# orhosko/tiny-ntt

Hardware: AMD Instinct MI355X
Metric: negacyclic poly-mults/sec (n=4096, 60-bit q), bit-exact vs cg_ntt.py (higher is better)
Workload: dtype u64; 1 GPU; n=4096, q=2^60-2^14+1 (60-bit), global batch 65536 = 65536 rows on this GPU, LCG-seeded rows resident in HBM (BASELINE configs[2]); n=4096, q=1152921504606830593, rows_per_gpu=65536, global_batch=65536, variant=fused, kernel=polymul_fused_kernel, lazy_reduction=True, lib_build_id=280bdc49742b142f, parallelism=batch-sharded x1, no data-path collective

## Files before the change

### __graft_entry__.py

```python
import ctypes
import os
import subprocess
import sys

ROOT = os.path.dirname(os.path.abspath(__file__))
REFERENCE = os.environ.get("TINY_NTT_REFERENCE", "/root/reference")


def _make(directory, *targets):
    cmd = ["make", f"-j{min(8, os.cpu_count() or 1)}", "-C", os.path.join(ROOT, directory), *targets]
    r = subprocess.run(cmd, stdout=subprocess.PIPE, stderr=subprocess.STDOUT, text=True)
    if r.returncode != 0:
        sys.stderr.write(r.stdout)
        raise RuntimeError(f"build failed: {' '.join(cmd)}")


def build() -> None:
    _make("tiny_ntt_amd/csrc")
    _make("oracle", "all")
    _make("tests/emu")
    _make("tests/emu_gadget2")
    _make("tests/devprobe")
    if os.path.isdir(os.path.join(REFERENCE, "software_benchmark")):
        _make("oracle", "ref", f"REFERENCE={REFERENCE}")
    sys.path.insert(0, ROOT)
    import tiny_ntt_amd
    from tiny_ntt_amd import engine
    lib = engine.load_library()
    missing = [s for s in engine.EXPORTED_SYMBOLS if not hasattr(lib, s)]
    if missing:
        raise RuntimeError(f"libtinyntt.so lacks symbols: {missing}")


def smoke() -> None:
    sys.path.insert(0, ROOT)
    import numpy as np
    from tiny_ntt_amd import engine

    n, q, psi = 4096, 1152921504606830593, 431606828070683274
    plan = engine.Plan(n, q, psi, device=0)
    rng = np.random.default_rng(7)
    batch = 4
    a = rng.integers(0, q, size=(batch, n), dtype=np.uint64)
    b = rng.integers(0, q, size=(batch, n), dtype=np.uint64)
    a[0, :] = q - 1
    c = plan.poly_mult(a, b)
    c_cg = plan.poly_mult(a, b, variant="cg8")

    so = os.path.join(ROOT, "oracle", "_build", "liboracle.so")
    if not os.path.exists(so):
        _make("oracle", "all")
    orc = ctypes.CDLL(so)
    P = ctypes.POINTER(ctypes.c_uint64)
    orc.tn_oracle_nwc_poly_mult_batch.argtypes = [P, P, P, ctypes.c_size_t, ctypes.c_size_t, ctypes.c_uint64, ctypes.c_uint64]
    ref = np.empty_like(a)
    rc = orc.tn_oracle_nwc_poly_mult_batch(a.ctypes.data_as(P), b.ctypes.data_as(P), ref.ctypes.data_as(P), batch, n, q, psi)
    assert rc == 0
    assert np.array_equal(c, ref), "fused kernel differs from the oracle"
    assert np.array_equal(c_cg, ref), "cg8 kernel differs from the oracle"
    print(f"smoke ok: n={n} q={q} batch={batch} fused(lazy={plan.is_lazy}) and cg8 bit-exact vs oracle")


if __name__ == "__main__":
    build()
    if len(sys.argv) > 1 and sys.argv[1] == "smoke":
        smoke()
```

### tiny_ntt_amd/csrc/fused_core.h

```cpp
#pragma once
#include <type_traits>
#include "modarith.h"

#ifndef TN_ABL_UNIFORM_TW
#define TN_ABL_UNIFORM_TW 0
#endif

namespace tn {

template <int B, int E_, typename F> struct StaticFor {
  TN_HD static void run(F& f) { f(std::integral_constant<int, B>()); StaticFor<B + 1, E_, F>::run(f); }
};
template <int E_, typename F> struct StaticFor<E_, E_, F> { TN_HD static void run(F&) {} };
template <int B, int E_, typename F> TN_HD void static_for(F&& f) { StaticFor<B, E_, F>::run(f); }

#ifndef TN_FUSED_LPT10
#define TN_FUSED_LPT10 3
#endif
#ifndef TN_FUSED_LPT12
#define TN_FUSED_LPT12 3
#endif
constexpr int fused_lpt(int logn) {
  return logn == 8 ? 2 : logn == 9 ? 3 : logn == 10 ? TN_FUSED_LPT10 : logn == 11 ? 3 : logn == 12 ? TN_FUSED_LPT12 : logn == 13 ? 3 : 0;
}

template <typename E> struct Arith {
  E q;
  u64 mu;
  int k;
  u32 fold_c;
  SplitK sk;
  u64 qmul[17];
  typename TwOf<E>::type one;
  typename TwOf<E>::type ninv;
  typename TwOf<E>::type fninv;
  typename TwOf<E>::type fninv_w1;
  typename TwOf<E>::type bninv;
  typename TwOf<E>::type bninv_w1;
};

template <typename E, int LOGN_, int LPT_> struct FusedCfg {
  static constexpr int LOGN = LOGN_, LPT = LPT_;
  static constexpr int N = 1 << LOGN, R = 1 << LPT, THREADS = N >> LPT;
  static constexpr int PHASES = (LOGN + LPT - 1) / LPT;
  static constexpr int pos(int p) { return (LOGN - (p + 1) * LPT) < 0 ? 0 : (LOGN - (p + 1) * LPT); }
  static constexpr int stage_begin(int p) { return p * LPT; }
  static constexpr int stage_end(int p) { return ((p + 1) * LPT) < LOGN ? ((p + 1) * LPT) : LOGN; }
  static constexpr int ex_pad(int e) { return pos(e + 1) > 0 ? (1 << pos(e + 1)) : 1; }
  static constexpr int ex_sh(int e) { return pos(e + 1) > 0 ? pos(e + 1) + LPT : LPT; }
  static constexpr int lay_span(int e, int cnt) { return cnt + ex_pad(e) * (cnt >> ex_sh(e)); }
  static constexpr int WB = (LOGN - LPT > 6) ? (LOGN - LPT - 6) : 0;
  static constexpr int WSH = LOGN - WB;
  static constexpr int tau_bit_to_j(int p, int t) { return t < pos(p) ? t : t + LPT; }
  static constexpr bool ex_wave_local(int e) {
    for (int t = 6; t < LOGN - LPT; ++t)
      if (tau_bit_to_j(e, t) != t + LPT || tau_bit_to_j(e + 1, t) != t + LPT) return false;
    return true;
  }
  static constexpr int region_elems() {
    int m = 1 << WSH;
    for (int e = 0; e + 1 < PHASES; ++e)
      if (ex_wave_local(e) && lay_span(e, 1 << WSH) > m) m = lay_span(e, 1 << WSH);
    return m;
  }
  static constexpr int lds_elems() {
    int m = region_elems() << WB;
    for (int e = 0; e + 1 < PHASES; ++e)
      if (!ex_wave_local(e) && lay_span(e, N) > m) m = lay_span(e, N);
    return m;
  }
  TN_HD static constexpr u32 jidx(int p, u32 tau, u32 r) {
    return ((tau >> pos(p)) << (pos(p) + LPT)) | (r << pos(p)) | (tau & ((1u << pos(p)) - 1u));
  }
  TN_HD static constexpr u32 prep_idx(u32 tau, u32 r) { return (r << (LOGN - LPT)) | tau; }
  TN_HD static constexpr u32 ex_addr(int e, u32 j) {
    if (WB > 0 && ex_wave_local(e))
      return (j >> WSH) * (u32)region_elems() + (j & ((1u << WSH) - 1u)) + (u32)ex_pad(e) * ((j & ((1u << WSH) - 1u)) >> ex_sh(e));
    return j + (u32)ex_pad(e) * (j >> ex_sh(e));
  }
  TN_HD static constexpr u32 ex_base(int e, int p, u32 tau) { return ex_addr(e, jidx(p, tau, 0)); }
  TN_HD static constexpr u32 ex_off(int e, int p, u32 r) { return ex_addr(e, jidx(p, 0, r)); }
  enum { TW_UNIFORM = 0, TW_WAVE = 1, TW_LDS = 2, TW_REGS = 3, TW_VEC = 4 };
  static constexpr int LDS_TW_MAX_STAGE = 9;
  static constexpr int tw_src(int p) {
    return pos(p) >= LOGN - LPT ? TW_UNIFORM
         : (pos(p) >= 6 ? TW_WAVE : (pos(p) > 0 ? (stage_end(p) <= LDS_TW_MAX_STAGE ? TW_LDS : TW_VEC) : TW_REGS));
  }
  static constexpr int lds_tw_lo() {
    for (int p = 0; p < PHASES; ++p) if (tw_src(p) == TW_LDS) return 1 << stage_begin(p);
    return 0;
  }
  static constexpr int lds_tw_hi() {
    int h = 0;
    for (int p = 0; p < PHASES; ++p) if (tw_src(p) == TW_LDS) h = 1 << stage_end(p);
    return h;
  }
  static constexpr int lds_tw_count() { return lds_tw_hi() - lds_tw_lo(); }
  static constexpr int pre_count(int s) { return R >> ((LOGN - 1 - s) - pos(PHASES - 1) + 1); }
  static constexpr int pre_off(int s) {
    int o = 0;
    for (int i = stage_begin(PHASES - 1); i < s; ++i) o += pre_count(i);
    return o;
  }
  static constexpr int NPRE = (tw_src(PHASES - 1) == TW_REGS) ? pre_off(LOGN) : 1;
  TN_HD static u32 nat_addr(u32 k) { return k ^ ((k >> 5) & 15u); }
  TN_HD static u32 thi(int p, u32 tau) {
    if (pos(p) >= LOGN - LPT) return 0u;
    if (pos(p) >= 6) return wave_uniform(tau >> pos(p));
    return tau >> pos(p);
  }
};

template <typename E> struct LazyTraits;
template <> struct LazyTraits<u64> { static constexpr int LIMIT = 16, TMUL = 4, PW = 2; };
template <> struct LazyTraits<u32> { static constexpr int LIMIT = 64, TMUL = 2, PW = 4; };

template <typename E, bool LAZY, bool CIN = false> struct Policy {
  typedef typename TwOf<E>::type Tw;
  static constexpr bool lazy = LAZY;
  static constexpr bool canonical_inputs = CIN && LAZY && sizeof(E) == 8;
  static constexpr bool split = LAZY && sizeof(E) == 8;
  static constexpr int LIMIT = LazyTraits<E>::LIMIT, TMUL = LazyTraits<E>::TMUL, PW = LazyTraits<E>::PW;

  TN_HD static E load(E x, const Arith<E>& ar) {
    if (canonical_inputs) return x;
    if (LAZY) return fold(x, ar.k, ar.fold_c);
    return mul_tw(x, ar.one, ar.q);
  }
  TN_HD static E canon(E x, const Arith<E>& ar) {
    if (LAZY) { x = fold(x, ar.k, ar.fold_c); return csub(x, ar.q); }
    return x;
  }
  template <int K> TN_HD static void ct(E& u, E& v, Tw w, const Arith<E>& ar) {
    if constexpr (split) {
      const u64 x = mul_sp_acc(u, v, w, ar.sk);
      v = ((u << 1) + ar.qmul[K]) - x;
      u = x;
    } else if constexpr (LAZY) {
      const E t = mul_tw_lazy(v, w, ar.q);
      v = u + ((E)K * ar.q - t);
      u = u + t;
    } else {
      E t = mul_tw(v, w, ar.q);
      E s = u + t;
      v = u >= t ? u - t : u + (ar.q - t);
      u = csub(s, ar.q);
    }
  }
  template <int BND> TN_HD static void gs(E& u, E& v, Tw w, const Arith<E>& ar) {
    if constexpr (split) {
      const E d = (u + ar.qmul[BND]) - v;
      u = u + v;
      v = mul_sp(d, w, ar.sk);
    } else if constexpr (LAZY) {
      const E d = u + ((E)BND * ar.q - v);
      u = u + v;
      v = mul_tw_lazy(d, w, ar.q);
    } else {
      E d = u >= v ? u - v : u + (ar.q - v);
      u = csub(u + v, ar.q);
      v = mul_tw(d, w, ar.q);
    }
  }
  template <int BND> TN_HD static void gs_last(E& u, E& v, const Arith<E>& ar) {
    E d;
    if constexpr (split) d = (u + ar.qmul[BND]) - v;
    else d = LAZY ? (E)(u + ((E)BND * ar.q - v)) : (u >= v ? (E)(u - v) : (E)(u + (ar.q - v)));
    E s = u + v;
    u = mul_tw_canon(s, ar.fninv, ar);
    v = mul_tw_canon(d, ar.fninv_w1, ar);
  }
  TN_HD static E mul_tw_canon(E a, Tw w, const Arith<E>& ar) {
    if constexpr (split) return csub(fold(mul_sp(a, w, ar.sk), ar.k, ar.fold_c), ar.q);
    else return mul_tw(a, w, ar.q);
  }
};

template <typename P, int LOGN> struct Sched {
  static constexpr int fwd_in(int s) {
    int b = 2;
    for (int i = 0; i < s; ++i) { if (b + P::TMUL > P::LIMIT) b = 2; b += P::TMUL; }
    return b;
  }
  static constexpr bool fwd_fold(int s) { return P::lazy && fwd_in(s) + P::TMUL > P::LIMIT; }
  static constexpr int fwd_out() {
    int b = 2;
    for (int i = 0; i < LOGN; ++i) { if (b + P::TMUL > P::LIMIT) b = 2; b += P::TMUL; }
    return b;
  }
  static constexpr int inv_in(int g) {
    int b = P::lazy ? P::PW : 1;
    for (int i = 0; i < g; ++i) { if (2 * b > P::LIMIT) b = 2; b = (2 * b > P::TMUL) ? 2 * b : P::TMUL; }
    return b;
  }
  static constexpr bool inv_fold(int g) { return P::lazy && 2 * inv_in(g) > P::LIMIT; }
  static constexpr int inv_bnd(int g) { return inv_fold(g) ? 2 : inv_in(g); }
};

template <typename Cfg, bool CIN = false, bool BC = false> struct SplitSched {
  static constexpr int LOGN = Cfg::LOGN, R = Cfg::R;
  static constexpr int FEND = BC ? LOGN - 1 : LOGN;
  static constexpr long U = 4096, CAP = 16 * U;
  static constexpr long FOLDED = U + 1;
  static constexpr long PW_OUT = 2 * U;
  static constexpr long PW_IN = 14 * (U - 1);
  static constexpr long tmax(long bv) { return 4 * U + (bv + 7) / 8 + 2; }
  static constexpr long BC_AMAX = CAP - 8;
  static constexpr int kq(long b) { return (int)((b + U - 2) / (U - 1)); }
  static constexpr int kf(long t) { return kq(t) <= 6 ? 6 : kq(t); }
  static constexpr int ki(long b) { return (kq(b) + 3) / 4 * 4; }
  static constexpr int phase_of(int s) { return s / Cfg::LPT; }
  static constexpr int bpos_of(int s) { return (LOGN - 1 - s) - Cfg::pos(phase_of(s)); }
  struct Data {
    bool ffold[LOGN][R] = {};
    unsigned char fk[LOGN][R] = {};
    long fout = 0;
    bool pw_fold_b = false;
    bool bcfold[R] = {};
    bool ifold[LOGN][R] = {};
    unsigned char ik[LOGN][R] = {};
  };
  static constexpr Data build() {
    Data d;
    long b[R] = {};
    for (int r = 0; r < R; ++r) b[r] = CIN ? U : (r < R / 2 ? FOLDED : CAP);
    for (int s = 0; s < FEND; ++s) {
      if (s > 0 && phase_of(s) != phase_of(s - 1)) {
        long m = 0;
        for (int r = 0; r < R; ++r) m = b[r] > m ? b[r] : m;
        for (int r = 0; r < R; ++r) b[r] = m;
      }
      const int bit = 1 << bpos_of(s);
      for (int r = 0; r < R; ++r) {
        if (r & bit) continue;
// ... 325 lines not shown
```

### tiny_ntt_amd/csrc/fused_kernels.h

```cpp
#pragma once
#include <hip/hip_runtime.h>
#include <type_traits>
#include "plan.h"
#include "dev_addr.h"

#ifndef TN_ABL_NO_BARRIER
#define TN_ABL_NO_BARRIER 0
#endif
#ifndef TN_ABL_ROWMASK
#define TN_ABL_ROWMASK 0
#endif
#ifndef TN_ABL_NO_GLOBAL
#define TN_ABL_NO_GLOBAL 0
#endif
#ifndef TN_STORE_AT_TOP
#define TN_STORE_AT_TOP 1
#endif
#ifndef TN_NT_STREAM
#define TN_NT_STREAM 1
#endif
#ifndef TN_FUSED_MIN_WAVES
#define TN_FUSED_MIN_WAVES 4
#endif
#ifndef TN_POLYMUL60_WAVES
#define TN_POLYMUL60_WAVES 6
#endif

#ifndef TN_NTTF_PIN_LOGN
#define TN_NTTF_PIN_LOGN 99
#endif
#ifndef TN_VEC_PREFETCH
#define TN_VEC_PREFETCH 1
#endif
#ifndef TN_FUSED_CIN
#define TN_FUSED_CIN 0
#endif
#ifndef TN_SADDR
#define TN_SADDR 1
#endif
#ifndef TN_KARG_ARITH
#define TN_KARG_ARITH 1
#endif
#ifndef TN_RESIDENT_TW
#define TN_RESIDENT_TW 1
#endif
#ifndef TN_SHARE_MID_TW
#define TN_SHARE_MID_TW 1
#endif
#ifndef TN_SHARE_LAST_TW
#define TN_SHARE_LAST_TW 1
#endif
#ifdef TN_MARKS
#define TN_MARK(n) asm volatile("; TNMARK " n)
#else
#define TN_MARK(n)
#endif
namespace tn {

#ifndef TN_SHUFFLE_LAST
#define TN_SHUFFLE_LAST 0
#endif
template <int DIST> __device__ __forceinline__ u32 lane_xor(u32 v) {
  if constexpr (DIST == 1) return (u32)__builtin_amdgcn_update_dpp(0, (int)v, 0xB1, 0xf, 0xf, false);
  else if constexpr (DIST == 2) return (u32)__builtin_amdgcn_update_dpp(0, (int)v, 0x4E, 0xf, 0xf, false);
  else {
    int r = __builtin_amdgcn_update_dpp(0, (int)v, 0x104, 0xf, 0x5, false);
    return (u32)__builtin_amdgcn_update_dpp(r, (int)v, 0x114, 0xf, 0xA, false);
  }
}
template <typename E>
__device__ __forceinline__ void transpose8_lanes(E (&x)[8], u32 lane) {
  static_for<0, 3>([&](auto b_) {
    constexpr int b = decltype(b_)::value, m = 1 << b;
    const bool hi = (lane >> b) & 1u;
    static_for<0, 8>([&](auto r_) {
      constexpr int r0 = decltype(r_)::value;
      if constexpr (!(r0 & m)) {
        constexpr int r1 = r0 | m;
        const E send = hi ? x[r0] : x[r1];
        E recv;
        if constexpr (sizeof(E) == 8) recv = ((u64)lane_xor<m>((u32)(send >> 32)) << 32) | lane_xor<m>((u32)send);
        else recv = lane_xor<m>((u32)send);
        x[r0] = hi ? recv : x[r0];
        x[r1] = hi ? x[r1] : recv;
      }
    });
  });
}

template <typename E, typename Cfg, int EX, int FROM, int TO>
__device__ __forceinline__ void exchange(E (&x)[Cfg::R], u32 tau, E* lds) {
  if constexpr (TN_SHUFFLE_LAST && Cfg::LPT == 3 && EX == Cfg::PHASES - 2 && Cfg::pos(EX + 1) == 0 && Cfg::pos(EX) == Cfg::LPT) {
    transpose8_lanes<E>(x, tau);
  } else if constexpr (Cfg::ex_wave_local(EX)) {
    __builtin_amdgcn_wave_barrier();
    ex_store<E, Cfg, EX, FROM>(x, tau, lds);
    __builtin_amdgcn_wave_barrier();
    ex_load<E, Cfg, EX, TO>(x, tau, lds);
    __builtin_amdgcn_wave_barrier();
  } else {
#if TN_ABL_NO_BARRIER
    __builtin_amdgcn_wave_barrier();
    ex_store<E, Cfg, EX, FROM>(x, tau, lds);
    __builtin_amdgcn_wave_barrier();
    ex_load<E, Cfg, EX, TO>(x, tau, lds);
    __builtin_amdgcn_wave_barrier();
#else
    __syncthreads();
    ex_store<E, Cfg, EX, FROM>(x, tau, lds);
    __syncthreads();
    ex_load<E, Cfg, EX, TO>(x, tau, lds);
    __syncthreads();
#endif
  }
}

template <typename E>
__device__ __forceinline__ const Arith<E>& kernarg_arith(u32 zero) {
  typedef const __attribute__((address_space(4))) char* KP;
  return *(const Arith<E>*)((KP)__builtin_amdgcn_kernarg_segment_ptr() + zero);
}

template <typename E, typename Cfg, typename Pol, int P0, int P1, bool KARG = false, int PRE_END = Cfg::LOGN, bool BC = false>
__device__ __forceinline__ void forward_range(E (&x)[Cfg::R], u32 tau, const TwRefs<E>& tw_in, const Arith<E>& ar_in, E* lds, bool fetch_pre,
                                              u32 tau_g) {
  typename TwOf<E>::type vec[Cfg::R];
  static_for<P0, P1>([&](auto p_) {
    constexpr int p = decltype(p_)::value;
    constexpr bool FULL = Cfg::stage_end(p) - Cfg::stage_begin(p) == Cfg::LPT;
    TN_MARK("fwd_phase");
    TwRefs<E> tw = tw_in;
    if constexpr (KARG) tw.zero = opaque_zero();
    if constexpr (TN_VEC_PREFETCH && Cfg::tw_src(p) == Cfg::TW_VEC && FULL && p > P0) tw.mid = vec;
    const Arith<E>& ar = KARG ? kernarg_arith<E>(tw.zero) : ar_in;
    fwd_phase<E, Cfg, Pol, p, BC>(x, tau, tw, ar);
    TN_MARK("fwd_other");
    if constexpr (p == Cfg::PHASES - 2) {
      if (fetch_pre) {
        sched_fence();
        tw_prefetch_stages<E, Cfg, Cfg::stage_begin(Cfg::PHASES - 1), PRE_END>(tw.pre, tau_g, tw.glob);
        sched_fence();
      }
    }
    if constexpr (p + 1 < P1) {
      constexpr int pn = p + 1 < Cfg::PHASES ? p + 1 : p;
      if constexpr (TN_VEC_PREFETCH && Cfg::tw_src(pn) == Cfg::TW_VEC && Cfg::stage_end(pn) - Cfg::stage_begin(pn) == Cfg::LPT) {
        sched_fence();
        tw_fetch_vec<E, Cfg, pn>(vec, tau_g, tw.glob);
        sched_fence();
      }
    }
    if constexpr (p + 1 < Cfg::PHASES) exchange<E, Cfg, p, p, p + 1>(x, tau, lds);
  });
}
template <typename E, typename Cfg, typename Pol>
__device__ __forceinline__ void forward_all(E (&x)[Cfg::R], u32 tau, const typename TwOf<E>::type* __restrict__ glob,
                                            const typename TwOf<E>::type* lds_tw, const Arith<E>& ar, E* lds, u32 zero = 0) {
  typename TwOf<E>::type pre[Cfg::NPRE];
  const TwRefs<E> tw = {glob, lds_tw, pre, nullptr, zero};
  forward_range<E, Cfg, Pol, 0, Cfg::PHASES>(x, tau, tw, ar, lds, true, tau);
}

template <typename E, typename Cfg, typename Pol, bool KARG = false, bool BC = false, typename F>
__device__ __forceinline__ void inverse_all(E (&x)[Cfg::R], u32 tau, const TwRefs<E>& tw_in, const Arith<E>& ar_in, E* lds,
                                            F&& after_first) {
  typename TwOf<E>::type vec[Cfg::R];
  static_for<0, Cfg::PHASES>([&](auto i_) {
    constexpr int p = Cfg::PHASES - 1 - decltype(i_)::value;
    constexpr bool FULL = Cfg::stage_end(p) - Cfg::stage_begin(p) == Cfg::LPT;
    TN_MARK("inv_phase");
    TwRefs<E> tw = tw_in;
    if constexpr (KARG) tw.zero = opaque_zero();
    if constexpr (TN_VEC_PREFETCH && Cfg::tw_src(p) == Cfg::TW_VEC && FULL && p < Cfg::PHASES - 1) tw.mid = vec;
    const Arith<E>& ar = KARG ? kernarg_arith<E>(tw.zero) : ar_in;
    inv_phase<E, Cfg, Pol, p, BC>(x, tau, tw, ar);
    TN_MARK("inv_other");
    if constexpr (p > 0) {
      constexpr int pn = p > 0 ? p - 1 : 0;
      if constexpr (TN_VEC_PREFETCH && Cfg::tw_src(pn) == Cfg::TW_VEC && Cfg::stage_end(pn) - Cfg::stage_begin(pn) == Cfg::LPT) {
        sched_fence();
        tw_fetch_vec<E, Cfg, pn>(vec, tau, tw.glob);
        sched_fence();
      }
    }
    if constexpr (p == Cfg::PHASES - 1) { sched_fence(); after_first(); sched_fence(); }
    if constexpr (p > 0) exchange<E, Cfg, p - 1, p, p - 1>(x, tau, lds);
  });
}

template <typename E> struct alignas(2 * sizeof(E)) PairOf { E lo, hi; };

template <typename E, typename Cfg>
__device__ __forceinline__ E ld_operand(const E* __restrict__ p, u32 row, u32 tau, int r) {
#if TN_ABL_NO_GLOBAL
  return (E)(tau * 2654435761u + 7 * r + row);
#else
#if TN_ABL_ROWMASK
  row &= TN_ABL_ROWMASK;
#endif
#if TN_NT_STREAM
  const TN_GLOBAL_AS E* rp = uniform_ptr(p + ((size_t)row << Cfg::LOGN) + Cfg::jidx(0, 0, r));
  return __builtin_nontemporal_load(rp + (Cfg::jidx(0, tau, 0) & (u32)(Cfg::N - 1)));
#else
  return p[((size_t)row << Cfg::LOGN) + Cfg::jidx(0, tau, r)];
#endif
#endif
}

template <typename E, typename Cfg>
__device__ __forceinline__ void st_result(E* __restrict__ c, u32 row, u32 tau, const E (&x)[Cfg::R]) {
#if TN_ABL_ROWMASK
  row &= TN_ABL_ROWMASK;
#endif
  const size_t off = (size_t)row << Cfg::LOGN;
#pragma unroll
  for (int r = 0; r < Cfg::R; ++r) {
#if TN_NT_STREAM
    __builtin_nontemporal_store(x[r], uniform_ptr(c + off + Cfg::jidx(0, 0, r)) + (Cfg::jidx(0, tau, 0) & (u32)(Cfg::N - 1)));
#else
    c[off + Cfg::jidx(0, tau, r)] = x[r];
#endif
  }
}

template <typename E, typename Cfg, bool NT>
__device__ __forceinline__ E ld_prepared(const E* __restrict__ p, u32 row, u32 tau, int r) {
  if constexpr (NT && TN_NT_STREAM) {
    const TN_GLOBAL_AS E* rp = uniform_ptr(p + ((size_t)row << Cfg::LOGN) + Cfg::prep_idx(0, r));
    return __builtin_nontemporal_load(rp + Cfg::prep_idx(tau, 0));
  } else {
    return p[((size_t)row << Cfg::LOGN) + Cfg::prep_idx(tau, r)];
  }
}

template <typename E, int LOGN, int LPT, bool LAZY>
constexpr int polymul_waves() {
  return LPT >= 4 ? 2 : (sizeof(E) == 8 && LOGN == 12 && LAZY) ? TN_POLYMUL60_WAVES : TN_FUSED_MIN_WAVES;
}
#ifndef TN_DOT_WAVES
#define TN_DOT_WAVES 4
#endif
template <typename E, int LOGN, int LPT, bool LAZY>
constexpr int dot_waves() {
  return polymul_waves<E, LOGN, LPT, LAZY>() > TN_DOT_WAVES ? TN_DOT_WAVES : polymul_waves<E, LOGN, LPT, LAZY>();
}

__device__ __forceinline__ void take_next_row(u32& left, u32& chunk_id, u32* lds_next, u32 slot, u32 cur, u32* sched, u32 chunk) {
  if (left) { --left; lds_next[slot] = cur + 1; }
  else {
    chunk_id = sched ? gridDim.x + atomicAdd(&sched[0], 1u) : chunk_id + gridDim.x;
    left = chunk - 1;
    lds_next[slot] = chunk_id * chunk;
  }
}

__device__ __forceinline__ void rearm_row_counters(u32* sched, u32 tau) {
  if (sched && tau == 0 && atomicAdd(&sched[1], 1u) == gridDim.x - 1) { sched[0] = 0; sched[1] = 0; }
}

template <typename E, typename Cfg, typename Pol, bool BC>
__device__ __forceinline__ void dot_last_term(E (&acc)[Cfg::R], E (&xa)[Cfg::R], const E (&xb)[Cfg::R], const typename TwOf<E>::type* zeta,
                                              typename TwOf<E>::type (&pre)[Cfg::NPRE], u32 tl, const typename TwOf<E>::type* tab_inv,
                                              const Arith<E>& ar) {
  if constexpr (BC) {
    basecase<Cfg, Pol>(xa, xb, zeta, ar);
    sched_fence();
    tw_prefetch_stages<E, Cfg, Cfg::stage_begin(Cfg::PHASES - 1), Cfg::LOGN - 1>(pre, tl, tab_inv);
  } else {
    tw_prefetch<E, Cfg>(pre, tl, tab_inv);
    pointwise<E, Cfg, Pol>(xa, xb, ar);
  }
  dot_accumulate<E, Cfg, Pol>(acc, xa, ar);
}

template <bool PRODUCT = false, typename F>
inline hipError_t dispatch_fused_shape(const tn_plan* p, F&& f) {
#ifdef TN_ONLY_MAIN
  if constexpr (PRODUCT) { if (p->elem_bytes == 8 && p->lazy && p->logn == 12) return f(FusedShape<u64, 12, true>()); }
  return hipErrorInvalidValue;
#else
  return with_fused_shape(p->elem_bytes, p->lazy, p->logn, hipErrorInvalidValue, f);
#endif
}

template <typename Sh> struct FusedProductLaunch {
  typedef typename Sh::E E;
  typedef typename TwOf<E>::type Tw;
  static constexpr bool HAS_BC = Sh::HAS_BC;
  const PlanView<E> pv;
  const bool use_bc;
  const FusedProductSetup<E> su;
  explicit FusedProductLaunch(const tn_plan* p, bool cyclic = false, bool no_bc = false)
      : pv(make_view<E>(p)), use_bc(fused_use_bc<Sh>(p->bc_ok, no_bc)), su(fused_product_setup(pv.ar, use_bc, cyclic)) {}
  const Tw* fwd() const { return fused_table(pv, su.fwd); }
  const Tw* inv() const { return fused_table(pv, su.inv); }
};

template <typename Sh>
constexpr size_t fused_lds_bytes(int tables, size_t extra_elems = 0) {
  typedef typename Sh::Cfg Cfg;
  return ((size_t)Cfg::lds_elems() + extra_elems) * sizeof(typename Sh::E) + (size_t)tables * Cfg::lds_tw_count() * sizeof(typename TwOf<typename Sh::E>::type) + 16;
}

}
```

### tiny_ntt_amd/csrc/kernels.hip

```cpp
#include "fused_kernels.h"

namespace tn {

#ifdef TN_FUSED_STAMPS
__device__ unsigned long long tn_fused_stamps[4 * 4096];
#endif

template <typename E, int LOGN, int LPT, bool LAZY, bool CIN = false, bool BC = false>
__global__ void __launch_bounds__((1 << (LOGN - LPT)), (polymul_waves<E, LOGN, LPT, LAZY>()))
polymul_fused_kernel(const Arith<E> ar, const typename TwOf<E>::type* __restrict__ tab_fwd,
                     const typename TwOf<E>::type* __restrict__ tab_inv, const E* __restrict__ a, const E* __restrict__ b,
                     E* __restrict__ c, u32 batch, u32* sched, u32 chunk) {
  typedef FusedCfg<E, LOGN, LPT> Cfg;
  typedef Policy<E, LAZY, CIN> Pol;
  extern __shared__ __attribute__((aligned(16))) unsigned char tn_smem[];
  typedef typename TwOf<E>::type Tw;
  const u32 tau = threadIdx.x;
  E* lds = reinterpret_cast<E*>(tn_smem);
  Tw* lds_fwd = reinterpret_cast<Tw*>(lds + Cfg::lds_elems());
  Tw* lds_inv = lds_fwd + Cfg::lds_tw_count();
  u32* lds_next = reinterpret_cast<u32*>(lds_inv + Cfg::lds_tw_count());
  for (u32 i = tau; i < (u32)Cfg::lds_tw_count(); i += Cfg::THREADS) {
    lds_fwd[i] = tab_fwd[Cfg::lds_tw_lo() + i];
    lds_inv[i] = tab_inv[Cfg::lds_tw_lo() + i];
  }
  __syncthreads();
  E xa[Cfg::R], xb[Cfg::R];
#ifdef TN_FUSED_STAMPS
  const unsigned long long st_t0 = __builtin_amdgcn_s_memtime(), st_r0 = __builtin_amdgcn_s_memrealtime();
#endif
  u32 row = blockIdx.x * chunk;
  u32 taken = 1;
  u32 chunk_id = blockIdx.x;
  if (row < batch) {
#pragma unroll
    for (int r = 0; r < Cfg::R; ++r) xb[r] = ld_operand<E, Cfg>(a, row, tau, r);
  }
  constexpr int PRE_END = (TN_RESIDENT_TW && polymul_waves<E, LOGN, LPT, LAZY>() <= 4 && Cfg::stage_end(Cfg::PHASES - 1) - Cfg::stage_begin(Cfg::PHASES - 1) >= 2) ? Cfg::LOGN - 1 : Cfg::LOGN;
  Tw prf[Cfg::NPRE];
  tw_prefetch_stages<E, Cfg, PRE_END, Cfg::LOGN>(prf, tau, tab_fwd);
  u32 prev = row;
  bool have_c = false;
#pragma unroll
  for (int r = 0; r < Cfg::R; ++r) xa[r] = 0;
  while (row < batch) {
    const u32 zero = opaque_zero();
    const u32 tl = opaque_copy(tau);
    const bool in_chunk = taken != chunk;
    taken = in_chunk ? taken + 1 : 1;
    chunk_id = in_chunk ? chunk_id : chunk_id + gridDim.x;
    if (tau == 0) *lds_next = in_chunk ? row + 1 : (sched ? gridDim.x + atomicAdd(&sched[0], 1u) : chunk_id) * chunk;
    TN_MARK("loop_top");
    E xn[Cfg::R];
#pragma unroll
    for (int r = 0; r < Cfg::R; ++r) xn[r] = xb[r];
    load_reduce<E, Cfg, Pol>(xn, ar);
    sched_fence();
#if TN_STORE_AT_TOP
    st_result<E, Cfg>(c, prev, tl, xa);
#endif
#pragma unroll
    for (int r = 0; r < Cfg::R; ++r) xb[r] = ld_operand<E, Cfg>(b, row, tl, r);
    sched_fence();
#pragma unroll
    for (int r = 0; r < Cfg::R; ++r) xa[r] = xn[r];
    constexpr bool KARG = TN_KARG_ARITH != 0;
    constexpr bool SHARE = TN_SHARE_LAST_TW && Cfg::PHASES >= 2;
    constexpr int PM = Cfg::PHASES >= 3 ? Cfg::PHASES - 2 : 0;
    constexpr bool SHARE2 = SHARE && TN_SHARE_MID_TW && Cfg::PHASES >= 3 && Cfg::tw_src(PM) == Cfg::TW_LDS &&
                            Cfg::stage_end(PM) - Cfg::stage_begin(PM) == Cfg::LPT;
    const TwRefs<E> twf = {tab_fwd, lds_fwd, prf, nullptr, zero};
    static_assert(!BC || SHARE2, "base case: built for the shared-twiddle schedule only");
    if constexpr (SHARE2) forward_range<E, Cfg, Pol, 0, PM, KARG, Cfg::LOGN, BC>(xa, tau, twf, ar, lds, false, tl);
    else if constexpr (SHARE) forward_range<E, Cfg, Pol, 0, Cfg::PHASES - 1, KARG>(xa, tau, twf, ar, lds, false, tl);
    else forward_all<E, Cfg, Pol>(xa, tau, tab_fwd, lds_fwd, ar, lds, zero);
    __syncthreads();
    const u32 next = wave_uniform(*lds_next);
    load_reduce<E, Cfg, Pol>(xb, ar);
    if constexpr (SHARE2) {
      forward_range<E, Cfg, Pol, 0, PM, KARG, Cfg::LOGN, BC>(xb, tau, twf, ar, lds, false, tl);
      Tw mid[Cfg::R];
      tw_fetch_mid<E, Cfg, PM>(mid, tau, lds_fwd);
      const TwRefs<E> twm = {tab_fwd, lds_fwd, prf, mid, zero};
      forward_range<E, Cfg, Pol, PM, PM + 1, KARG, Cfg::LOGN, BC>(xa, tau, twm, ar, lds, false, tl);
      forward_range<E, Cfg, Pol, PM, PM + 1, KARG, PRE_END, BC>(xb, tau, twm, ar, lds, true, tl);
      forward_range<E, Cfg, Pol, PM + 1, Cfg::PHASES, KARG, Cfg::LOGN, BC>(xb, tau, twf, ar, lds, false, tl);
      forward_range<E, Cfg, Pol, PM + 1, Cfg::PHASES, KARG, Cfg::LOGN, BC>(xa, tau, twf, ar, lds, false, tl);
    } else if constexpr (SHARE) {
      forward_range<E, Cfg, Pol, 0, Cfg::PHASES - 1, KARG, PRE_END>(xb, tau, twf, ar, lds, true, tl);
      forward_range<E, Cfg, Pol, Cfg::PHASES - 1, Cfg::PHASES, KARG>(xb, tau, twf, ar, lds, false, tl);
      forward_range<E, Cfg, Pol, Cfg::PHASES - 1, Cfg::PHASES, KARG>(xa, tau, twf, ar, lds, false, tl);
    } else {
      forward_all<E, Cfg, Pol>(xb, tau, tab_fwd, lds_fwd, ar, lds, zero);
    }
    Tw pre[Cfg::NPRE];
    if constexpr (BC) {
      TN_MARK("basecase");
      basecase<Cfg, Pol>(xa, xb, prf + Cfg::pre_off(Cfg::LOGN - 1), ar);
      sched_fence();
      tw_prefetch_stages<E, Cfg, Cfg::stage_begin(Cfg::PHASES - 1), Cfg::LOGN - 1>(pre, tl, tab_inv);
    } else {
      tw_prefetch<E, Cfg>(pre, tl, tab_inv);
      TN_MARK("pointwise");
      pointwise<E, Cfg, Pol>(xa, xb, ar);
    }
    TN_MARK("after_pointwise");
    const TwRefs<E> twi = {tab_inv, lds_inv, pre, nullptr, zero};
    inverse_all<E, Cfg, Pol, KARG, BC>(xa, tau, twi, ar, lds, [&]() {
      const u32 nrow = next < batch ? next : row;
#pragma unroll
      for (int r = 0; r < Cfg::R; ++r) xb[r] = ld_operand<E, Cfg>(a, nrow, tl, r);
    });
#if TN_STORE_AT_TOP
    prev = row;
    have_c = true;
#else
    st_result<E, Cfg>(c, row, tau, xa);
#endif
    row = next;
  }
  if (have_c) st_result<E, Cfg>(c, prev, tau, xa);
#ifdef TN_FUSED_STAMPS
  if (tau == 0 && blockIdx.x < 4096) {
    tn_fused_stamps[4 * blockIdx.x + 0] = st_t0; tn_fused_stamps[4 * blockIdx.x + 1] = st_r0;
    tn_fused_stamps[4 * blockIdx.x + 2] = __builtin_amdgcn_s_memtime(); tn_fused_stamps[4 * blockIdx.x + 3] = __builtin_amdgcn_s_memrealtime();
  }
#endif
  rearm_row_counters(sched, tau);
}

template <typename E, int LOGN, int LPT, bool LAZY, int MODE>
__global__ void __launch_bounds__((1 << (LOGN - LPT)), (LPT >= 4 ? 2 : TN_FUSED_MIN_WAVES))
ntt_fused_kernel(const Arith<E> ar, const typename TwOf<E>::type* __restrict__ tab, const E* __restrict__ in, E* __restrict__ out, u32 batch,
                 u32* sched, u32 chunk) {
  typedef FusedCfg<E, LOGN, LPT> Cfg;
  typedef Policy<E, LAZY> Pol;
  typedef typename TwOf<E>::type Tw;
  extern __shared__ __attribute__((aligned(16))) unsigned char tn_smem[];
  E* lds = reinterpret_cast<E*>(tn_smem);
  const u32 tau = threadIdx.x;
  E* nat = lds + Cfg::lds_elems();
  Tw* lds_tab = reinterpret_cast<Tw*>(nat + Cfg::N);
  u32* lds_next = reinterpret_cast<u32*>(lds_tab + Cfg::lds_tw_count());
  for (u32 i = tau; i < (u32)Cfg::lds_tw_count(); i += Cfg::THREADS) lds_tab[i] = tab[Cfg::lds_tw_lo() + i];
  u32 left = chunk - 1, chunk_id = blockIdx.x;
  if (tau == 0) take_next_row(left, chunk_id, lds_next, 1u, blockIdx.x * chunk, sched, chunk);
  __syncthreads();
  u32 next = wave_uniform(lds_next[1]);
  constexpr int LAST = Cfg::PHASES - 1;
  E xn[Cfg::R];
  u32 row = blockIdx.x * chunk;
  if (row < batch) {
#pragma unroll
    for (int r = 0; r < Cfg::R; ++r) xn[r] = ld_operand<E, Cfg>(in, row, tau, r);
  }
  for (u32 it = 0; row < batch; ++it) {
    if (tau == 0) take_next_row(left, chunk_id, lds_next, it & 1u, next, sched, chunk);
    constexpr bool PIN = LOGN >= TN_NTTF_PIN_LOGN;
    const u32 zero = PIN ? opaque_zero() : 0u;
    const u32 tl = PIN ? opaque_copy(tau) : tau;
    constexpr bool KARG = PIN && TN_KARG_ARITH != 0;
    E x[Cfg::R];
#pragma unroll
    for (int r = 0; r < Cfg::R; ++r) x[r] = xn[r];
    sched_fence();
    if (MODE != FNTT_CYCLIC_INV && next < batch) {
#pragma unroll
      for (int r = 0; r < Cfg::R; ++r) xn[r] = ld_operand<E, Cfg>(in, next, tl, r);
    }
    sched_fence();
    if (MODE == FNTT_CYCLIC_INV) {
#pragma unroll
      for (int r = 0; r < Cfg::R; ++r) x[r] = Pol::load(x[r], ar);
#pragma unroll
      for (int r = 0; r < Cfg::R; ++r) nat[Cfg::nat_addr(Cfg::jidx(0, tau, r))] = x[r];
      __syncthreads();
#pragma unroll
      for (int r = 0; r < Cfg::R; ++r) x[r] = nat[Cfg::nat_addr(bitrev(Cfg::jidx(LAST, tau, r), LOGN))];
      Tw pre[Cfg::NPRE];
      tw_prefetch<E, Cfg>(pre, tl, tab);
      const TwRefs<E> tw = {tab, lds_tab, pre, nullptr, zero};
      inverse_all<E, Cfg, Pol, KARG>(x, tau, tw, ar, lds, [&]() {
        if (next < batch) {
#pragma unroll
          for (int r = 0; r < Cfg::R; ++r) xn[r] = ld_operand<E, Cfg>(in, next, tl, r);
        }
      });
      st_result<E, Cfg>(out, row, tl, x);
    } else {
#pragma unroll
      for (int r = 0; r < Cfg::R / 2; ++r) x[r] = Pol::load(x[r], ar);
      if (!LAZY) {
#pragma unroll
        for (int r = Cfg::R / 2; r < Cfg::R; ++r) x[r] = Pol::load(x[r], ar);
      }
      {
        Tw pre[Cfg::NPRE];
        const TwRefs<E> tw = {tab, lds_tab, pre, nullptr, zero};
        forward_range<E, Cfg, Pol, 0, Cfg::PHASES, KARG>(x, tau, tw, ar, lds, true, tl);
      }
#pragma unroll
      for (int r = 0; r < Cfg::R; ++r)
        nat[Cfg::nat_addr(bitrev(Cfg::jidx(LAST, tau, r), LOGN))] = LAZY ? Pol::canon(x[r], ar) : x[r];
      __syncthreads();
#pragma unroll
      for (int r = 0; r < Cfg::R; ++r) x[r] = nat[Cfg::nat_addr(Cfg::jidx(0, tau, r))];
      st_result<E, Cfg>(out, row, tl, x);
    }
    if (Cfg::THREADS <= 64) __syncthreads();
    row = next;
    next = wave_uniform(lds_next[it & 1u]);
  }
  rearm_row_counters(sched, tau);
}

template <typename Sh>
static hipError_t launch_nttf_t(const tn_plan* p, int mode, const void* in, void* out, size_t batch, hipStream_t s) {
  typedef typename Sh::E E;
  typedef typename Sh::Cfg Cfg;
  typedef typename TwOf<E>::type Tw;
  constexpr int LOGN = Sh::LOGN, LPT = Sh::LPT;
  constexpr bool LAZY = Sh::LAZY;
  constexpr size_t lds_bytes = fused_lds_bytes<Sh>(1, Cfg::N);
  const PlanView<E> pv = make_view<E>(p);
  auto kern = ntt_fused_kernel<E, LOGN, LPT, LAZY, FNTT_TWIST_FWD>;
  if (mode == FNTT_CYCLIC_FWD) kern = ntt_fused_kernel<E, LOGN, LPT, LAZY, FNTT_CYCLIC_FWD>;
  else if (mode != FNTT_TWIST_FWD) kern = ntt_fused_kernel<E, LOGN, LPT, LAZY, FNTT_CYCLIC_INV>;
  const FusedNttSetup<E> su = fused_ntt_setup(pv.ar, mode);
  return launch_persistent(p, s, (const void*)kern, Cfg::THREADS, lds_bytes, Cfg::N * sizeof(E), batch, FUSED_ROWS, [&](u32 grid, u32* sched, u32 chunk) {
    const Tw* tab = fused_table(pv, su.tab);
    const E* in_ = (const E*)in; E* out_ = (E*)out; u32 b32 = (u32)batch;
    Arith<E> ar = su.ar;
    void* args[] = {&ar, &tab, &in_, &out_, &b32, &sched, &chunk};
    return hipLaunchKernel((const void*)kern, dim3(grid), dim3(Cfg::THREADS), args, lds_bytes, s);
  });
}

hipError_t launch_ntt_fused(const tn_plan* p, int mode, const void* in, void* out, size_t batch, hipStream_t s) {
  if (batch == 0) return hipSuccess;
  return dispatch_fused_shape(p, [&](auto sh) { return launch_nttf_t<decltype(sh)>(p, mode, in, out, batch, s); });
}

bool fused_supported(u32 logn, int) { return fused_lpt((int)logn) != 0; }

template <typename Sh>
static hipError_t launch_fused_t(const tn_plan* p, const void* a, const void* b, void* c, size_t batch, hipStream_t s, bool cyclic) {
  typedef typename Sh::E E;
  typedef typename Sh::Cfg Cfg;
  constexpr int LOGN = Sh::LOGN, LPT = Sh::LPT;
  constexpr bool LAZY = Sh::LAZY;
  constexpr size_t lds_bytes = fused_lds_bytes<Sh>(2);
  constexpr bool HAS_CIN = TN_FUSED_CIN && sizeof(E) == 8 && LOGN == 12 && LAZY;
  const bool use_cin = HAS_CIN && p->canonical_inputs && !cyclic;
  const FusedProductLaunch<Sh> L(p, cyclic, use_cin);
  auto kern = polymul_fused_kernel<E, LOGN, LPT, LAZY>;
  if constexpr (HAS_CIN) { if (use_cin) kern = polymul_fused_kernel<E, LOGN, LPT, LAZY, true>; }
  if constexpr (L.HAS_BC) { if (L.use_bc) kern = polymul_fused_kernel<E, LOGN, LPT, LAZY, false, true>; }
  return launch_persistent(p, s, reinterpret_cast<const void*>(kern), Cfg::THREADS, lds_bytes, Cfg::N * sizeof(E), batch, FUSED_ROWS,
                           [&](u32 grid, u32* sched, u32 chunk) {
    hipLaunchKernelGGL(kern, dim3(grid), dim3(Cfg::THREADS), lds_bytes, s, L.su.ar, L.fwd(), L.inv(),
                       (const E*)a, (const E*)b, (E*)c, (u32)batch, sched, chunk);
// ... 183 lines not shown
```

Before: 30.12 million poly-mults/s.

## Drop redundant block barriers around cross-wave LDS transposes in polymul row

```diff
diff --git a/__graft_entry__.py b/__graft_entry__.py
--- a/__graft_entry__.py
+++ b/__graft_entry__.py
@@ -20,6 +20,7 @@
     _make("oracle", "all")
     _make("tests/emu")
     _make("tests/emu_gadget2")
+    _make("tests/emu_sync")
     _make("tests/devprobe")
     if os.path.isdir(os.path.join(REFERENCE, "software_benchmark")):
         _make("oracle", "ref", f"REFERENCE={REFERENCE}")
diff --git a/tiny_ntt_amd/csrc/fused_core.h b/tiny_ntt_amd/csrc/fused_core.h
--- a/tiny_ntt_amd/csrc/fused_core.h
+++ b/tiny_ntt_amd/csrc/fused_core.h
@@ -6,6 +6,9 @@
 #define TN_ABL_UNIFORM_TW 0
 #endif
 
+#ifndef TN_PRODUCT_SYNC
+#define TN_PRODUCT_SYNC 1
+#endif
 namespace tn {
 
 template <int B, int E_, typename F> struct StaticFor {
@@ -80,6 +83,53 @@
   }
   TN_HD static constexpr u32 ex_base(int e, int p, u32 tau) { return ex_addr(e, jidx(p, tau, 0)); }
   TN_HD static constexpr u32 ex_off(int e, int p, u32 r) { return ex_addr(e, jidx(p, 0, r)); }
+  enum { EXB_BEFORE = 1, EXB_BETWEEN = 2, EXB_AFTER = 4, EXB_ALL = 7 };
+  static constexpr bool side_region_local_eval(int e, int p) {
+    const bool local = WB > 0 && ex_wave_local(e);
+    const u32 region = (u32)region_elems(), pad = (u32)ex_pad(e), low = (1u << WSH) - 1u;
+    const int sh = ex_sh(e);
+    for (u32 tau = 0; tau < (u32)THREADS; ++tau)
+      for (u32 r = 0; r < (u32)R; ++r) {
+        const u32 j = jidx(p, tau, r), w = tau >> 6;
+        const u32 a = local ? (j >> WSH) * region + (j & low) + pad * ((j & low) >> sh) : j + pad * (j >> sh);
+        if (a < w * region || a >= (w + 1) * region) return false;
+      }
+    return true;
+  }
+  template <int EX, bool TO> static constexpr bool SIDE_REGION_LOCAL = side_region_local_eval(EX, EX + (TO ? 1 : 0));
+  static constexpr bool ex_from_region_local(int e) {
+    return e == 0 ? SIDE_REGION_LOCAL<0, false> : e == 1 ? SIDE_REGION_LOCAL<1, false> : e == 2 ? SIDE_REGION_LOCAL<2, false>
+         : e == 3 ? SIDE_REGION_LOCAL<3, false> : side_region_local_eval(e, e);
+  }
+  static constexpr bool ex_to_region_local(int e) {
+    return e == 0 ? SIDE_REGION_LOCAL<0, true> : e == 1 ? SIDE_REGION_LOCAL<1, true> : e == 2 ? SIDE_REGION_LOCAL<2, true>
+         : e == 3 ? SIDE_REGION_LOCAL<3, true> : side_region_local_eval(e, e + 1);
+  }
+  static constexpr int last_cross_ex() {
+    int l = -1;
+    for (int e = 0; e + 1 < PHASES; ++e) if (!ex_wave_local(e)) l = e;
+    return l;
+  }
+  static constexpr int prod_fwd_barriers(int e, bool first = false) {
+    return (ex_to_region_local(e) ? (EXB_BEFORE | EXB_BETWEEN) : EXB_ALL) & ~(first && e == 0 ? EXB_BEFORE : 0);
+  }
+  static constexpr int prod_inv_barriers(int e) { return (e == last_cross_ex() && ex_to_region_local(e)) ? EXB_BETWEEN : EXB_ALL; }
+  static constexpr bool prod_sync_ok() {
+    const int L = last_cross_ex();
+    for (int e = 0; e + 1 < PHASES; ++e) {
+      if (ex_wave_local(e) != (e > L)) return false;
+      if (ex_wave_local(e)) {
+        if (WB > 0 && !(ex_from_region_local(e) && ex_to_region_local(e))) return false;
+        continue;
+      }
+      const int f = prod_fwd_barriers(e), i = prod_inv_barriers(e);
+      if (!(f & EXB_BEFORE) || !(f & EXB_BETWEEN) || !(i & EXB_BETWEEN)) return false;
+      if (!(f & EXB_AFTER) && !ex_to_region_local(e)) return false;
+      if (!(i & EXB_BEFORE) && !(e == L && ex_to_region_local(e))) return false;
+      if (!(i & EXB_AFTER) && e > 0 && !(prod_inv_barriers(e - 1) & EXB_BEFORE)) return false;
+    }
+    return (region_elems() << WB) <= lds_elems();
+  }
   enum { TW_UNIFORM = 0, TW_WAVE = 1, TW_LDS = 2, TW_REGS = 3, TW_VEC = 4 };
   static constexpr int LDS_TW_MAX_STAGE = 9;
   static constexpr int tw_src(int p) {
diff --git a/tiny_ntt_amd/csrc/fused_kernels.h b/tiny_ntt_amd/csrc/fused_kernels.h
--- a/tiny_ntt_amd/csrc/fused_kernels.h
+++ b/tiny_ntt_amd/csrc/fused_kernels.h
@@ -88,7 +88,7 @@
   });
 }
 
-template <typename E, typename Cfg, int EX, int FROM, int TO>
+template <typename E, typename Cfg, int EX, int FROM, int TO, int BAR = Cfg::EXB_ALL>
 __device__ __forceinline__ void exchange(E (&x)[Cfg::R], u32 tau, E* lds) {
   if constexpr (TN_SHUFFLE_LAST && Cfg::LPT == 3 && EX == Cfg::PHASES - 2 && Cfg::pos(EX + 1) == 0 && Cfg::pos(EX) == Cfg::LPT) {
     transpose8_lanes<E>(x, tau);
@@ -106,11 +106,12 @@
     ex_load<E, Cfg, EX, TO>(x, tau, lds);
     __builtin_amdgcn_wave_barrier();
 #else
-    __syncthreads();
+    static_assert(BAR & Cfg::EXB_BETWEEN, "a cross-wave transpose always has the barrier between its stores and its loads");
+    if constexpr (BAR & Cfg::EXB_BEFORE) __syncthreads(); else __builtin_amdgcn_wave_barrier();
     ex_store<E, Cfg, EX, FROM>(x, tau, lds);
     __syncthreads();
     ex_load<E, Cfg, EX, TO>(x, tau, lds);
-    __syncthreads();
+    if constexpr (BAR & Cfg::EXB_AFTER) __syncthreads(); else __builtin_amdgcn_wave_barrier();
 #endif
   }
 }
@@ -121,7 +122,7 @@
   return *(const Arith<E>*)((KP)__builtin_amdgcn_kernarg_segment_ptr() + zero);
 }
 
-template <typename E, typename Cfg, typename Pol, int P0, int P1, bool KARG = false, int PRE_END = Cfg::LOGN, bool BC = false>
+template <typename E, typename Cfg, typename Pol, int P0, int P1, bool KARG = false, int PRE_END = Cfg::LOGN, bool BC = false, int PSYNC = 0>
 __device__ __forceinline__ void forward_range(E (&x)[Cfg::R], u32 tau, const TwRefs<E>& tw_in, const Arith<E>& ar_in, E* lds, bool fetch_pre,
                                               u32 tau_g) {
   typename TwOf<E>::type vec[Cfg::R];
@@ -150,7 +151,7 @@
         sched_fence();
       }
     }
-    if constexpr (p + 1 < Cfg::PHASES) exchange<E, Cfg, p, p, p + 1>(x, tau, lds);
+    if constexpr (p + 1 < Cfg::PHASES) exchange<E, Cfg, p, p, p + 1, PSYNC ? Cfg::prod_fwd_barriers(p, PSYNC == 1) : Cfg::EXB_ALL>(x, tau, lds);
   });
 }
 template <typename E, typename Cfg, typename Pol>
@@ -161,7 +162,7 @@
   forward_range<E, Cfg, Pol, 0, Cfg::PHASES>(x, tau, tw, ar, lds, true, tau);
 }
 
-template <typename E, typename Cfg, typename Pol, bool KARG = false, bool BC = false, typename F>
+template <typename E, typename Cfg, typename Pol, bool KARG = false, bool BC = false, bool PSYNC = false, typename F>
 __device__ __forceinline__ void inverse_all(E (&x)[Cfg::R], u32 tau, const TwRefs<E>& tw_in, const Arith<E>& ar_in, E* lds,
                                             F&& after_first) {
   typename TwOf<E>::type vec[Cfg::R];
@@ -184,7 +185,7 @@
       }
     }
     if constexpr (p == Cfg::PHASES - 1) { sched_fence(); after_first(); sched_fence(); }
-    if constexpr (p > 0) exchange<E, Cfg, p - 1, p, p - 1>(x, tau, lds);
+    if constexpr (p > 0) exchange<E, Cfg, p - 1, p, p - 1, PSYNC ? Cfg::prod_inv_barriers(p - 1) : Cfg::EXB_ALL>(x, tau, lds);
   });
 }
 
diff --git a/tiny_ntt_amd/csrc/kernels.hip b/tiny_ntt_amd/csrc/kernels.hip
--- a/tiny_ntt_amd/csrc/kernels.hip
+++ b/tiny_ntt_amd/csrc/kernels.hip
@@ -70,15 +70,23 @@
     constexpr bool SHARE2 = SHARE && TN_SHARE_MID_TW && Cfg::PHASES >= 3 && Cfg::tw_src(PM) == Cfg::TW_LDS &&
                             Cfg::stage_end(PM) - Cfg::stage_begin(PM) == Cfg::LPT;
     const TwRefs<E> twf = {tab_fwd, lds_fwd, prf, nullptr, zero};
+    constexpr bool PSYNC = TN_PRODUCT_SYNC != 0 && SHARE && Cfg::last_cross_ex() >= 0;
+    static_assert(!PSYNC || Cfg::prod_sync_ok(), "product row: a barrier was left out where its argument does not hold");
+    static_assert(!PSYNC || !SHARE2 || Cfg::ex_wave_local(PM), "product row: a and b interleave only behind the cross-wave transposes");
+    static_assert(!PSYNC || !(LOGN == 12 && LPT == 3) ||
+                  (Cfg::last_cross_ex() == 0 && Cfg::ex_to_region_local(0) && !Cfg::ex_from_region_local(0) && Cfg::region_elems() == 576 &&
+                   Cfg::prod_fwd_barriers(0, true) == Cfg::EXB_BETWEEN && Cfg::prod_fwd_barriers(0, false) == (Cfg::EXB_BEFORE | Cfg::EXB_BETWEEN) &&
+                   Cfg::prod_inv_barriers(0) == Cfg::EXB_BETWEEN),
+                  "n = 4096: four barriers per row");
     static_assert(!BC || SHARE2, "base case: built for the shared-twiddle schedule only");
-    if constexpr (SHARE2) forward_range<E, Cfg, Pol, 0, PM, KARG, Cfg::LOGN, BC>(xa, tau, twf, ar, lds, false, tl);
-    else if constexpr (SHARE) forward_range<E, Cfg, Pol, 0, Cfg::PHASES - 1, KARG>(xa, tau, twf, ar, lds, false, tl);
+    if constexpr (SHARE2) forward_range<E, Cfg, Pol, 0, PM, KARG, Cfg::LOGN, BC, PSYNC ? 1 : 0>(xa, tau, twf, ar, lds, false, tl);
+    else if constexpr (SHARE) forward_range<E, Cfg, Pol, 0, Cfg::PHASES - 1, KARG, Cfg::LOGN, false, PSYNC ? 1 : 0>(xa, tau, twf, ar, lds, false, tl);
     else forward_all<E, Cfg, Pol>(xa, tau, tab_fwd, lds_fwd, ar, lds, zero);
-    __syncthreads();
+    if constexpr (!PSYNC) __syncthreads();
     const u32 next = wave_uniform(*lds_next);
     load_reduce<E, Cfg, Pol>(xb, ar);
     if constexpr (SHARE2) {
-      forward_range<E, Cfg, Pol, 0, PM, KARG, Cfg::LOGN, BC>(xb, tau, twf, ar, lds, false, tl);
+      forward_range<E, Cfg, Pol, 0, PM, KARG, Cfg::LOGN, BC, PSYNC ? 2 : 0>(xb, tau, twf, ar, lds, false, tl);
       Tw mid[Cfg::R];
       tw_fetch_mid<E, Cfg, PM>(mid, tau, lds_fwd);
       const TwRefs<E> twm = {tab_fwd, lds_fwd, prf, mid, zero};
@@ -87,7 +95,7 @@
       forward_range<E, Cfg, Pol, PM + 1, Cfg::PHASES, KARG, Cfg::LOGN, BC>(xb, tau, twf, ar, lds, false, tl);
       forward_range<E, Cfg, Pol, PM + 1, Cfg::PHASES, KARG, Cfg::LOGN, BC>(xa, tau, twf, ar, lds, false, tl);
     } else if constexpr (SHARE) {
-      forward_range<E, Cfg, Pol, 0, Cfg::PHASES - 1, KARG, PRE_END>(xb, tau, twf, ar, lds, true, tl);
+      forward_range<E, Cfg, Pol, 0, Cfg::PHASES - 1, KARG, PRE_END, false, PSYNC ? 2 : 0>(xb, tau, twf, ar, lds, true, tl);
       forward_range<E, Cfg, Pol, Cfg::PHASES - 1, Cfg::PHASES, KARG>(xb, tau, twf, ar, lds, false, tl);
       forward_range<E, Cfg, Pol, Cfg::PHASES - 1, Cfg::PHASES, KARG>(xa, tau, twf, ar, lds, false, tl);
     } else {
@@ -106,7 +114,7 @@
     }
     TN_MARK("after_pointwise");
     const TwRefs<E> twi = {tab_inv, lds_inv, pre, nullptr, zero};
-    inverse_all<E, Cfg, Pol, KARG, BC>(xa, tau, twi, ar, lds, [&]() {
+    inverse_all<E, Cfg, Pol, KARG, BC, PSYNC>(xa, tau, twi, ar, lds, [&]() {
       const u32 nrow = next < batch ? next : row;
 #pragma unroll
       for (int r = 0; r < Cfg::R; ++r) xb[r] = ld_operand<E, Cfg>(a, nrow, tl, r);
```

Measured after the change: 30.39 million poly-mults/s, median of 6. No clear change (+0.9%).
